# RoboEden/flatland-marl

Hardware: AMD Instinct MI355X
Metric: agent-steps/sec (batched envs) + tree-obs build ms/step (higher is better)
Workload: dtype int32; 1 GPU; cfg2: 256 envs x 30x30 / 20 agents / 3 cities (Round-2 Test_2); envs_per_gpu=256, agents=20, obs=cutils(31 nodes, pred 500) + upstream tree depth 2 (pred 30), actions=counter-hash uniform 0..4 generated on device, auto-reset at episode end, distinct_maps=8, dm_rebuild=at commit only, parallelism=envs sharded over 1 GPU(s), metrics all-reduce only, launch=one host call per kernel launch

## Files before the change

### flatland_marl_amd/csrc/fl_obs.hip

```cpp
#include <algorithm>
#include <stdio.h>
#include <stdlib.h>
#include <string.h>

#include "../../include/flatland_hip.h"
#include "fl_obs_layout.h"

int fl_obs_alloc(FlObsScratch &o, const FlDev &d, hipStream_t s, std::vector<void *> &allocs) {
    o.pred_cap = OBS_PRED_CAP;
    o.items_cap = (size_t)d.A * (o.pred_cap + 2 * OBS_FB_NB + 2);
    o.wl_cap = OBS_WL_HBM_ENTRIES;
    const size_t B = (size_t)d.B, BA = B * d.A;
    if (fl_alloc_zeroed(&o.path, BA * o.pred_cap, s, allocs) != hipSuccess ||
        fl_alloc_zeroed(&o.cell_items, B * o.items_cap, s, allocs, 64) != hipSuccess ||
        fl_alloc_zeroed(&o.dbg, B * 64, s, allocs) != hipSuccess || fl_alloc_zeroed(&o.bk_rel, B * (d.Rcap + 1) * OBS_BK_NB, s, allocs) != hipSuccess ||
        fl_alloc_zeroed(&o.wl, B * o.wl_cap, s, allocs) != hipSuccess || fl_alloc_zeroed(&o.label, (size_t)d.A, s, allocs) != hipSuccess ||
        fl_alloc_zeroed(&o.rowmask, BA, s, allocs) != hipSuccess || fl_alloc_zeroed(&o.cost, B, s, allocs) != hipSuccess ||
        fl_alloc_zeroed(&o.order, B, s, allocs) != hipSuccess) return FL_ERR_HIP;
    o.rows_out = nullptr; o.rows_depth = 0; o.keep_rows = 0;
    int dev = 0, n_cu = 0;
    if (hipGetDevice(&dev) != hipSuccess || hipDeviceGetAttribute(&n_cu, hipDeviceAttributeMultiprocessorCount, dev) != hipSuccess) return FL_ERR_HIP;
    o.n_cu = n_cu;
    o.order_age = 0;
    return FL_OK;
}

bool fl_obs_no_compact() { static const bool v = getenv("FL_OBS_NO_COMPACT") != nullptr; return v; }
static bool obs_no_fix() { static const bool v = getenv("FL_OBS_NO_FIX") != nullptr; return v; }
static bool obs_no_split() { static const bool v = getenv("FL_OBS_NO_SPLIT") != nullptr; return v; }
static bool obs_no_cutils_merge() { static const bool v = getenv("FL_OBS_NO_CUTILS_MERGE") != nullptr; return v; }
static bool obs_verbose_on() { static const bool v = getenv("FL_OBS_VERBOSE") != nullptr; return v; }
static bool obs_no_wl_head() { static const bool v = getenv("FL_OBS_NO_WL_HEAD") != nullptr; return v; }

__global__ __launch_bounds__(1024) void k_env_order(int B, const uint32_t *__restrict__ cost, int *__restrict__ order) {
    __shared__ unsigned int hist[1024];
    __shared__ unsigned int wsum[16];
    __shared__ unsigned int cmax;
    const int tid = threadIdx.x;
    hist[tid] = 0;
    if (tid == 0) cmax = 1;
    __syncthreads();
    unsigned int m = 0;
    for (int b = tid; b < B; b += 1024) m = max(m, cost[b]);
    for (int off = 32; off > 0; off >>= 1) m = max(m, (unsigned int)__shfl_down((int)m, off));
    if ((tid & 63) == 0) atomicMax(&cmax, m);
    __syncthreads();
// ... 375 lines not shown
    record[0] = -1;
    return d.A <= 1024 && pred_depth + 2 <= o.pred_cap && pred_depth <= 510;
}
static int obs_run(FlObsScratch &o, const FlDev &d, ObsArgs &P, const int *h_R, hipStream_t s, int record[FL_OBS_LAUNCH_WORDS]) {
    ObsOptions accepted = {};
    const int n_fit = obs_configure(d, P, accepted, h_R);
    if (n_fit < 0) return FL_ERR_ARG;
    o.last_fix = P.fix; o.last_split = P.split; o.last_fit = n_fit;
    uint4 *const rowmask = o.rowmask;
    struct Restore { FlObsScratch &o; uint4 *m; ~Restore() { o.rowmask = m; } } restore{o, rowmask};
    if (P.tw_t) {
        P.keep_rows = o.keep_rows && o.rows_out == P.tree_out && o.rows_depth == P.max_depth;
        o.rows_out = P.tree_out; o.rows_depth = P.max_depth;
        if (!o.keep_rows || P.max_depth > 3) { o.rowmask = nullptr; P.keep_rows = 0; o.rows_out = nullptr; }
    }
    obs_verbose(P);
    obs_keep_verify(d, P, rowmask, s);
    FlObsScratch u = o;
    if (P.merged == 1) u.order = nullptr;
    else u = fl_obs_env_order(o, d, s);
    const int rc = obs_launch(d, u, P, s);
    if (rc == FL_OK) obs_record_launch(P, accepted, record);
    return rc;
}

int fl_launch_obs_cutils(FlObsScratch &o, const FlDev &d, int max_nodes, int pred_depth, const FlObsCutilsOut &out, hipStream_t s,
                         int record[FL_OBS_LAUNCH_WORDS], const int16_t *label_dev, int out64) {
    if (!obs_begin(o, d, pred_depth, record) || max_nodes > FL_OBS_MAX_NODES) return FL_ERR_ARG;
    ObsArgs P = {};
    P.label = label_dev;
// ... 31 lines not shown

int fl_obs_config_of_fused(const FlDev &d, int pred_depth, int max_depth, int tree_pred, int out[11], int wide) {
    ObsArgs P = {};
    obs_cutils_args(P, 31, pred_depth, wide);
    if (max_depth > 0) obs_tree_args(d, P, max_depth, tree_pred, nullptr);
    else obs_alone_args(d, P);
    ObsOptions q = {};
    if (obs_configure(d, P, q, nullptr) < 0) return FL_ERR_ARG;
    if (obs_verbose_on()) {
        fprintf(stderr, "  options {nt %d, wl_bytes %d, tab %d, nh %d, tmask %d, dual %d, items %d, snext %d, partial %d, bk_room %d, own_filter %d, fb %d, raw %d, items_cap %d, wl_head %d}; "
                        "shape {merged %d, tw_c %d, tw_t %d, tpw_t %d, tree_pred %d}; bk %d tshift %d wl_occ_div %d\n",
                q.nt, q.wl_bytes, q.tab, q.nh, q.tmask, q.dual, q.items, q.snext, q.partial, q.bk_room, q.own_filter, q.fb, q.raw, q.items_cap, q.wl_head,
                P.merged, P.tw_c, P.tw_t, P.tpw_t, P.tree_pred, P.bk, P.tshift, P.wl_occ_div);
        static const char *names[L_COUNT] = {"cellw", "nbr", "snext", "rkey", "slot_agent", "slot_ready", "cell_target", "a_speed", "a_vpos", "a_pos", "a_tslot",
            "a_target", "a_malf", "a_tpc", "a_tq", "a_tq2", "a_raw", "rtype", "a_lp", "a_n", "a_srank", "a_dir", "a_state", "a_free", "a_dead", "misc", "team_meta", "node_tables",
            "csr", "items", "wl", "partial", "tmask", "tmask2", "nh", "csr2", "tmaskb", "tmaskb2", "items2", "a_lp2", "a_tpc2", "bkrel", "seg", "dm", "hop8"};
        for (int k = 0; k < L_COUNT; k++) {
            if (P.L.off[k] == L_ABSENT) continue;
            unsigned next = P.L.total;
            for (int j = 0; j < L_COUNT; j++) if (P.L.off[j] != L_ABSENT && P.L.off[j] > P.L.off[k] && P.L.off[j] < next) next = P.L.off[j];
            fprintf(stderr, "  %-12s %7u B\n", names[k], next - P.L.off[k]);
        }
    }
    out[0] = P.L.nt; out[1] = (int)P.L.total; out[2] = P.L.tab_lds; out[3] = P.L.off[L_NH] != L_ABSENT; out[4] = P.L.wl_bytes;
    out[5] = P.use_tmask + 2 * (P.L.off[L_TMASK2] != L_ABSENT);
    out[6] = P.dual_index; out[7] = P.L.off[L_ITEMS] != L_ABSENT ? P.L.items_cap : 0;
    out[8] = P.merged; out[9] = P.compact_t; out[10] = P.fix;
    return FL_OK;
}
```

### flatland_marl_amd/csrc/fl_obs_body.h

```cpp
#pragma once
#include "fl_obs_trees.h"

__device__ __forceinline__ int obs_env_of_workgroup(const FlObsScratch &S) { return __builtin_amdgcn_readfirstlane(S.order ? S.order[blockIdx.x] : (int)blockIdx.x); }

template <bool CUTILS, int VAR, int STAGE, int MERGED = 0, int FIX = 0, bool UP = true>
__device__ __forceinline__ void obs_body(const FlDev &d, const FlObsScratch &S, const ObsArgs &P_launch) {
    using FixT = ObsFixed<FIX != 0 ? FIX : 1>;
    ObsArgs P_local = P_launch;
    if (FIX != 0) {
        P_local.max_nodes = FixT::max_nodes; P_local.pred_depth = FixT::pred_depth; P_local.tree_pred = FixT::shape.tree_pred;
        P_local.tshift = obs_fixed_tshift<FIX != 0 ? FIX : 1>(d.A);
        if (FixT::max_depth != 0) {
            P_local.max_depth = FixT::max_depth;
            P_local.n_tree_nodes = FixT::max_depth == 2 ? 21 : 85;
        }
    }
    const ObsArgs &P = P_local;
    constexpr bool TAB_LDS = (VAR & 1) != 0, WL_HBM = (VAR & 2) != 0;
    const int b = MERGED == 1 ? (int)blockIdx.x : obs_env_of_workgroup(S), tid = threadIdx.x,
              nt = MERGED == 3 ? 512 : (FIX != 0 || MERGED == 1 || MERGED == 2) ? OBS_NT : (int)blockDim.x;
    const int A = (FIX != 0 && FixT::agents != 0) ? FixT::agents : d.A, R = d.R[b], NS = R * 4, K = d.K[b], U = d.U[b];
    const int Rcap = d.Rcap, Scap = Rcap * 4;
    const int lane = tid & 63, wave = tid >> 6;

// ... 31 lines not shown
    uint8_t *a_dead = LDS_AT(uint8_t, L_A_DEAD);
    int *misc = LDS_AT(int, L_MISC);
    int *team_meta = LDS_AT(int, L_TEAM_META);
    int *wave_scr = LDS_AT(int, L_WAVE_SCR);
    int *csr = LDS_AT(int, L_CSR);
    uint32_t *items_lds = LDS_OPT(uint32_t, L_ITEMS);
    uint32_t *wl_lds = WL_HBM ? nullptr : LDS_AT(uint32_t, L_WL);
    int *partial = (WL_HBM || L_OFF(L_PARTIAL) != L_ABSENT) ? LDS_AT(int, L_PARTIAL) : reinterpret_cast<int *>(wl_lds);
    const int wl_entries = WL_HBM ? OBS_WL_HBM_ENTRIES : L_FIELD(wl_bytes) / 8;
    unsigned long long *tmask = LDS_OPT(unsigned long long, L_TMASK);
    uint16_t *nh_lds = LDS_OPT(uint16_t, L_NH);
    int *csr2 = LDS_OPT(int, L_CSR2);
    unsigned long long *tmaskb = LDS_OPT(unsigned long long, L_TMASKB);
    unsigned long long *tmask_m2 = LDS_OPT(unsigned long long, L_TMASK2), *tmaskb_m2 = LDS_OPT(unsigned long long, L_TMASKB2);
    uint32_t *items2 = LDS_OPT(uint32_t, L_ITEMS2);
    uint16_t *a_lp2 = LDS_OPT(uint16_t, L_A_LP2);
    uint16_t *a_tpc2 = LDS_OPT(uint16_t, L_A_TPC2);
    double *a_tq2 = LDS_OPT(double, L_A_TQ2);
    uint32_t *a_raw = LDS_OPT(uint32_t, L_A_RAW);
    uint8_t *rtype_lds = LDS_OPT(uint8_t, L_RTYPE);
    uint4 *seg_lds = TAB_LDS ? LDS_AT(uint4, L_SEG) : nullptr;
    uint16_t *dm_lds = TAB_LDS ? LDS_AT(uint16_t, L_DM) : nullptr;
    uint16_t *hop8_lds = TAB_LDS ? LDS_AT(uint16_t, L_HOP8) : nullptr;
    const int tb = __builtin_amdgcn_readfirstlane(d.tab[b]);
    const uint4 *gseg = d.seg + (size_t)tb * Scap;
    const uint16_t *gdm = d.dm + (size_t)tb * d.Ucap * Scap;
    const uint16_t *ghop8 = d.hop8 + (size_t)tb * d.Ucap * Scap;
    const uint16_t *gnh = d.nh + (size_t)tb * d.Ucap * Rcap;

    const int T = d.T[b], tnow = d.t[b];
// ... 134 lines not shown
    X.wl_cf = X.wl_occ + X.wl_occ_cap; X.wl_cf_cap = wl_entries - X.wl_occ_cap;
    {
        const int head_entries = (WL_HBM && MERGED != 0 && L_OFF(L_WL) != L_ABSENT) ? L_FIELD(wl_head) / 8 : 0;
        uint2 *head = head_entries > 0 ? LDS_AT(uint2, L_WL) : nullptr;
        X.wl_head_occ = head; X.wl_head_occ_n = head_entries / p_wl_occ_div;
        X.wl_head_cf = head + X.wl_head_occ_n; X.wl_head_cf_n = head_entries - X.wl_head_occ_n;
    }
    X.wl_cnt = misc + 8;
    X.long_lists = misc + 11;
    X.tshift = X.Tn <= 64 ? 0 : P.tshift;
    constexpr bool merged = MERGED != 0;
    constexpr int ROUND = MERGED == 3 ? 16 : 32;
    X.n_cu = ROUND; X.round_base = 0;
    X.u_csr_end = csr2; X.u_items = items2; X.u_tmask = tmaskb; X.a_tq2 = a_tq2;
    X.tmask_m2 = merged ? tmask_m2 : nullptr; X.u_tmask_m2 = tmaskb_m2;
    X.path = S.path + (size_t)b * A * OBS_PRED_CAP; X.pred_cap = OBS_PRED_CAP;
    X.a_lp = a_lp; X.a_lp2 = a_lp2; X.a_tpc2 = a_tpc2;
    X.u_Tn = P.tree_pred + 1; X.u_tshift = X.u_Tn <= 64 ? 0 : P.tshift;

    OBS_STAMP(1);
    auto phase1a = [&]() __attribute__((always_inline)) {
        if (A <= 64) {
            const int i = lane;
            bool active = false, fr = false;
            unsigned long long blockers = 0;
            if (i < A && is_on_map(a_state[i]) && !a_dead[i]) {
                active = true;
                const uint32_t bits = nibble(cw_bits(X, a_pos[i]), a_dir[i]);
                if (bits == 0) fr = true;
                for (uint32_t m = 0; m < 4; m++) {
// ... 204 lines not shown
    }
    OBS_STAMP(2);
    if (X.Tn > 0) {
        const bool dual = UP && CUTILS && STAGE == 1 && p_dual_index && P.tree_pred >= 0;
        const bool reuse = STAGE == 2 && p_dual_index && misc[4] != 0;
        const int Tn2 = P.tree_pred + 1, tshift2 = Tn2 <= 64 ? 0 : P.tshift;
        const bool bk = CUTILS && STAGE != 2 && p_bk != 0 && X.Tn > 64 && X.tmask != nullptr;
        const bool bk_lds = bk && p_bk == 2;
        const int bk_nb = p_bk_nb, bk_shift = p_bk_shift;
        const int bk_w = bk_lds ? bk_nb + 2 : bk_nb;
        uint32_t *bkc = bk_lds ? LDS_AT(uint32_t, L_BKREL) : reinterpret_cast<uint32_t *>(wave_scr);
        if (!reuse) {
            for (int k = tid; k <= K; k += nt) csr[k] = 0;
            if (tid == 0) misc[11] = 0;
            if (X.tmask) for (int k = tid; k <= K; k += nt) { tmask[k] = 0ull; if (X.tmask_m2) tmask_m2[k] = 0ull; }
            if (bk) for (int k = tid; k < (bk_lds ? K * bk_w / 2 : ((K + 1) * bk_nb + 1) / 2); k += nt) bkc[k] = 0u;
        }
        if (dual) for (int k = tid; k <= K; k += nt) { csr2[k] = 0; if (p_use_tmask) tmaskb[k] = 0ull; if (X.tmask_m2) tmaskb_m2[k] = 0ull; }
        if (STAGE != 2 && tid < 64) { team_meta[64 + tid] = 1; team_meta[192 + tid] = 1; }
        __syncthreads();
        const int pred_depth = my_pred_depth;
        if (STAGE != 2) {
        const int w_first = (nt >> 6) - nw_walk, wsel = wave - w_first;
        if (do_p1 && p1_beside_walk && wave == w_first - 1) {
            phase1a();
#ifdef FL_OBS_TIMING
            if (lane == 0) atomicMax((unsigned long long *)&X.dbg[20], (unsigned long long)wall_clock64());
#endif
        }
        if (wsel >= 0) __builtin_amdgcn_s_setprio(3);
        const int n_max = CUTILS ? pred_depth + 1 : max(pred_depth, 1);
        for (int base = 0; wsel >= 0 && base < A; base += 8 * nw_walk) {
            const int slot = lane >> 3, j = lane & 7;
// ... 399 lines not shown
                } else {
                    tlo = k * tpc;
                    span = tpc;
                }
                const bool to_end = k == lp || tlo + span - 1 >= tlast;
                const int key = key_of(X, (int)(w >> 2));
                if (X.tmask) {
                    const int b1 = tb_of(tlo, X.tshift), b2 = tb_of(to_end ? tlast : tlo + span - 1, X.tshift);
                    const unsigned long long bits = ((2ull << b2) - 1ull) & ~((1ull << b1) - 1ull);
                    if (X.tmask_m2) {
                        const unsigned long long seen = atomicOr(&tmask[key], bits);
                        if (seen & bits) atomicOr(&tmask_m2[key], seen & bits);
                    } else {
                        atomicOr(&tmask[key], bits);
                    }
                }
                const uint32_t item = IT_MAKE(lab ? (int)lab[i] : i, tlo, to_end, span, dprev, dnext, w & 3u);
                if (bk) {
                    const int thi = to_end ? tlast : tlo + span - 1;
                    int b1 = min(tlo >> bk_shift, bk_nb - 1), b2 = min(thi >> bk_shift, bk_nb - 1);
                    if (bk_lds && to_end) b1 = b2 = bk_nb;
                    for (int bb = b1; bb <= b2; bb++) {
                        const int kb = key * bk_w + bb;
                        const uint32_t old = atomicAdd(&bkc[kb >> 1], (kb & 1) ? 0x10000u : 1u);
                        csr_items[csr[key] + (int)((kb & 1) ? (old >> 16) : (old & 0xFFFFu))] = item;
                    }
                } else {
                    const int slot = atomicAdd(&csr[key], 1);
                    csr_items[slot] = item;
                }
                if (k <= lp2) {
                    const int tlo2 = k * tpc2, tlast2 = Tn2 - 1;
                    const bool to_end2 = k == lp2 || tlo2 + tpc2 - 1 >= tlast2;
                    const uint32_t dnext2 = k < lp2 ? dnext : (w & 3u);
                    if (p_use_tmask) {
                        const int b1 = tb_of(tlo2, tshift2), b2 = tb_of(to_end2 ? tlast2 : tlo2 + tpc2 - 1, tshift2);
                        const unsigned long long bits = ((2ull << b2) - 1ull) & ~((1ull << b1) - 1ull);
                        if (X.tmask_m2) {
                            const unsigned long long seen = atomicOr(&tmaskb[key], bits);
                            if (seen & bits) atomicOr(&tmaskb_m2[key], seen & bits);
                        } else {
                            atomicOr(&tmaskb[key], bits);
                        }
                    }
                    const int slot2 = atomicAdd(&csr2[key], 1);
                    items2[slot2] = IT_MAKE(i, tlo2, to_end2, tpc2, dprev, dnext2, w & 3u);
                }
            }
            }
        }
        __syncthreads();
#ifdef FL_OBS_TIMING
        if (STAGE != 2 && tid == 0) {
            P.dbg[(size_t)b * 64 + 57] = (long long)wall_clock64();
            int wp = 0;
            for (int i = 0; i < A; i++) wp += a_n[i];
            P.dbg[(size_t)b * 64 + 58] = misc[2];
// ... 86 lines not shown
```

### flatland_marl_amd/csrc/fl_obs_ctx.h

```cpp
#pragma once
#include <stdio.h>
#include <type_traits>

#include "../../include/flatland_hip.h"
#include "fl_obs_layout.h"

struct ObsCtx {
    int A, R;
    int SS;
    const uint32_t *cellw;
    const uint16_t *nbr;
    const uint16_t *snext;
    const uint16_t *rkey;
    const int *slot_agent;
    const int *slot_ready;
    const uint32_t *cell_target;
    const uint16_t *a_vpos;
    const uint8_t *a_dir, *a_state;
    const uint16_t *a_malf;
    const double *a_speed;
    const uint16_t *a_tpc;
    const double *a_tq;
    const uint16_t *a_tslot;
    const uint16_t *a_target;
// ... 13 lines not shown
    int wl_occ_cap, wl_cf_cap;
    uint2 *wl_head_occ, *wl_head_cf;
    int wl_head_occ_n, wl_head_cf_n;
    int *wl_cnt;
    const int *long_lists;
    const unsigned long long *tmask;
    int tshift;
    int n_cu;
    int round_base;
    const int *u_csr_end;
    const uint32_t *u_items;
    const unsigned long long *u_tmask;
    int u_Tn, u_tshift;
    const double *a_tq2;
    const unsigned long long *tmask_m2, *u_tmask_m2;
    const uint16_t *path;
    int pred_cap;
    const uint16_t *a_lp, *a_lp2, *a_tpc2;
    long long *dbg;
    int dbg_base;
};

#ifndef OBS_NT_LEVEL
#define OBS_NT_LEVEL 2
#endif
typedef float obs_f4_t __attribute__((ext_vector_type(4)));
typedef double obs_d2_t __attribute__((ext_vector_type(2)));
__device__ __forceinline__ void fill_store_d2(double *p, double a, double b) {
#if OBS_NT_LEVEL >= 1
    const obs_d2_t v = {a, b};
// ... 22 lines not shown
template <typename T>
__device__ __forceinline__ void out_store(T *p, T v) {
#if OBS_NT_LEVEL >= 3
    __builtin_nontemporal_store(v, p);
#else
    *p = v;
#endif
}

__device__ __forceinline__ int tb_of(int t, int ts) { return min(t >> ts, 63); }

__device__ __forceinline__ uint32_t cw_bits(const ObsCtx &X, int r) { return X.cellw[r] & 0xFFFFu; }
__device__ __forceinline__ uint32_t cw_slot(const ObsCtx &X, int r) { return X.cellw[r] >> 16; }
__device__ __forceinline__ uint32_t cw_load(const ObsCtx &X, int r) { return X.cellw[r]; }
__device__ __forceinline__ int key_of(const ObsCtx &X, int r) { return X.rkey ? (int)X.rkey[r] : r; }
template <int PB>
__device__ __forceinline__ bool pb_cu(const ObsCtx &X, int team) { return PB == 3 ? true : PB == 2 ? team < X.n_cu : PB == 1; }
template <int PB>
__device__ __forceinline__ int pb_handle(const ObsCtx &X, const int *team_meta, int team) {
    return PB == 3 ? X.round_base + team : PB == 2 ? X.round_base + (team < X.n_cu ? team : team - X.n_cu) : team_meta[128 + team];
}
template <int PB>
__device__ __forceinline__ int pt_of(const ObsCtx &X, bool cu, int handle, int tot) {
    if (PB == 2 && !cu) return (int)((double)tot * X.a_tq2[handle]);
    return cu ? (int)((float)tot * (float)X.a_tq[handle]) : (int)((double)tot * X.a_tq[handle]);
}
struct ListRange { int lo, n1, lo2, n; };
template <bool TWO>
__device__ __forceinline__ int list_index(const ListRange &R, int v) { return (TWO && v >= R.n1) ? R.lo2 + (v - R.n1) : R.lo + v; }
template <int PB>
// ... 114 lines not shown
```

### flatland_marl_amd/csrc/fl_obs_layout.h

```cpp
#pragma once
#include <stdint.h>

#include "fl_obs.h"

#define OBS_NT 1024
#ifndef CF_CHUNK_LDS
#define CF_CHUNK_LDS 16
#endif
#ifndef CF_CHUNK_HBM
#define CF_CHUNK_HBM 8
#endif
#ifndef CF_FIRST_HBM
#define CF_FIRST_HBM 8
#endif
#ifndef OBS_GLB_BATCH
#define OBS_GLB_BATCH 8
#endif
#ifndef OBS_WL_OCC_DIV
#define OBS_WL_OCC_DIV 6
#endif
#ifndef OBS_TSHIFT
#define OBS_TSHIFT 1
#endif
#ifndef CF_DIRECT
// ... 27 lines not shown
#define N_NONE 0xFFFFu
enum { ND_TARGET = 1, ND_SWITCH = 2, ND_DEAD_END = 4, ND_TERMINAL = 8, ND_ZERO = 16, ND_PHANTOM = 32  };

#define OBS_CAP_C 32
#define OBS_CAP_T_COMPACT 16

__host__ __device__ constexpr int obs_scr_words(int nwaves, int A, int tw_c, int tw_t, int tpw_t) {
    const int tpw_c = tw_c > N_WORDS_C * OBS_CAP_C ? 1 : 2;
    const int n_c = tpw_c * nwaves <= A ? tpw_c * nwaves : A + 1, n_t = tpw_t * nwaves <= A ? tpw_t * nwaves : A + 1;
    const int w_c = n_c * tw_c, w_t = n_t * tw_t;
    return w_c > w_t ? w_c : w_t;
}

enum { L_CELLW = 0, L_NBR, L_SNEXT, L_RKEY, L_SLOT_AGENT, L_SLOT_READY, L_CELL_TARGET, L_A_SPEED, L_A_VPOS, L_A_POS, L_A_TSLOT,
       L_A_TARGET, L_A_MALF, L_A_TPC, L_A_TQ, L_A_TQ2, L_A_RAW, L_RTYPE, L_A_LP, L_A_N, L_A_SRANK, L_A_DIR, L_A_STATE, L_A_FREE, L_A_DEAD, L_MISC, L_TEAM_META, L_WAVE_SCR,
       L_CSR, L_ITEMS, L_WL, L_PARTIAL, L_TMASK, L_TMASK2, L_NH, L_CSR2, L_TMASKB, L_TMASKB2, L_ITEMS2, L_A_LP2, L_A_TPC2, L_BKREL, L_SEG, L_DM, L_HOP8, L_COUNT };
#define L_ABSENT 0xFFFFFFFFu
struct ObsLayout {
    unsigned off[L_COUNT];
    unsigned total;
    int nt;
    int wl_bytes;
    int wl_head;
    int tab_lds;
    int items_cap, items2_cap;
};

struct ObsOptions { int nt, wl_bytes, tab, nh, tmask, dual, items, snext, partial, bk_room, own_filter, fb, raw, items_cap, wl_head; };
struct ObsDims { int Rcap, A, Ucap, rkey; };
struct ObsShape { int merged, tw_c, tw_t, tpw_t, tree_pred; };

__host__ __device__ constexpr unsigned obs_al16(unsigned long long bytes) { return (unsigned)((bytes + 15ull) & ~15ull); }
__host__ __device__ constexpr ObsLayout obs_layout_c(const ObsDims &d, const ObsShape &P, const ObsOptions &o) {
    ObsLayout L = {};
    for (int k = 0; k < L_COUNT; k++) L.off[k] = L_ABSENT;
    unsigned off = 0;
#define OBS_PUT(which, bytes) do { L.off[which] = off; off += obs_al16((unsigned long long)(bytes)); } while (0)
    const unsigned long long R = (unsigned long long)d.Rcap, NS = R * 4, A = (unsigned long long)d.A, K1 = R + 1, U = (unsigned long long)d.Ucap;
    OBS_PUT(L_CELLW, R * 4);
    OBS_PUT(L_NBR, NS * 2);
    if (o.snext) OBS_PUT(L_SNEXT, NS * 2);
    if (d.rkey) OBS_PUT(L_RKEY, R * 2);
    OBS_PUT(L_SLOT_AGENT, A * 4); OBS_PUT(L_SLOT_READY, A * 4);
    OBS_PUT(L_CELL_TARGET, ((R + 31) / 32) * 4);
    OBS_PUT(L_A_SPEED, A * 8); OBS_PUT(L_A_TQ, A * 8);
    if (P.merged && o.raw) { OBS_PUT(L_A_RAW, A * 32); OBS_PUT(L_RTYPE, R); }
// ... 16 lines not shown
    L.items2_cap = (int)(i2 < OBS_ITEMS2_CAP ? i2 : OBS_ITEMS2_CAP);
    if (o.items) OBS_PUT(L_ITEMS, (unsigned long long)L.items_cap * 4);
    if (o.wl_bytes) OBS_PUT(L_WL, o.wl_bytes);
    else if (o.wl_head) OBS_PUT(L_WL, o.wl_head);
    if (o.partial || !o.wl_bytes) OBS_PUT(L_PARTIAL, (unsigned long long)o.nt * 4);
    if (o.tmask) OBS_PUT(L_TMASK, K1 * 8);
    if (o.tmask && P.merged && o.own_filter) OBS_PUT(L_TMASK2, K1 * 8);
    if (o.dual) {
        OBS_PUT(L_CSR2, K1 * 4);
        if (o.tmask) OBS_PUT(L_TMASKB, K1 * 8);
        if (o.tmask && P.merged && o.own_filter) OBS_PUT(L_TMASKB2, K1 * 8);
        OBS_PUT(L_ITEMS2, (unsigned long long)(L.items2_cap > 4 ? L.items2_cap : 4) * 4);
        OBS_PUT(L_A_LP2, A * 2); OBS_PUT(L_A_TPC2, A * 2); OBS_PUT(L_A_TQ2, A * 8);
    }
    if (o.fb) OBS_PUT(L_BKREL, K1 * (OBS_FB_NB + 2) * 2);
    if (o.nh || o.tab) OBS_PUT(L_NH, U * R * 2);
    if (o.tab) { OBS_PUT(L_SEG, NS * 16); OBS_PUT(L_DM, U * NS * 2); OBS_PUT(L_HOP8, U * NS * 2); }
#undef OBS_PUT
    L.total = off;
    L.nt = o.nt; L.wl_bytes = o.wl_bytes; L.tab_lds = o.tab; L.wl_head = o.wl_bytes ? 0 : o.wl_head;
    return L;
}

#define OBS_FIX3_RCAP 680
#define OBS_FIX4_RCAP 2816
#define OBS_FIX4_A 432
#define OBS_FIX3_WL_HEAD (10 * 1024)
#ifndef OBS_WL_HEAD_MAX
#define OBS_WL_HEAD_MAX (32 * 1024)
#endif
// ... 166 lines not shown
    int32_t *adjacency, *node_order, *edge_order;
    uint8_t *valid;
    double *props;
    double *tree_out;
    int n_tree_nodes;
    long long *dbg;
    int tw_c, tw_t, tpw_t;
    int compact_t;
    int use_tmask;
    int tshift;
    int dual_index;
    int bk;
    int bk_nb, bk_shift;
    int merged;
    int wl_occ_div;
    int fix;
    const int16_t *label;
    int keep_mode;
    int keep_rows;
    int out64;
    int cutils_alone;
    int wide;
    int fix_allowed;
    const int *h_R;
    int split;
    ObsLayout L;
};

template <int MODE>
int fl_obs_launch_mode(int var, const FlDev &d, const FlObsScratch &o, const ObsArgs &P, hipStream_t s);
// ... 3 lines not shown
```

### flatland_marl_amd/csrc/fl_obs_passb.h

```cpp
#pragma once
#include "fl_obs_ctx.h"

__device__ __forceinline__ void occ_event(const ObsCtx &X, bool CUTILS, int *sc, int cap, int node, uint32_t sl, uint32_t d, int tot) {
    const int ag = X.slot_agent[sl];
    if (ag < 0) return;
    atomicMin(&nt_w(sc, cap, N_OA, node), tot);
    const int mf = (int)X.a_malf[ag];
    if (mf > 0) {
        if (CUTILS) atomicOr(&nt_w(sc, cap, N_RM, node), 1 << 16);
        else atomicMax(&nt_w(sc, cap, N_MALF, node), mf);
    }
    const int rd = X.slot_ready[sl];
    const int radd = rd > 0 ? (CUTILS ? rd - 1 : rd) : 0;
    if (radd) atomicAdd(&nt_w(sc, cap, N_RM, node), radd);
    if (X.a_dir[ag] == d) {
        atomicAdd(&nt_w(sc, cap, N_CNT, node), 1);
        const double sp = CUTILS ? (double)(float)X.a_speed[ag] : X.a_speed[ag];
        if (sp < 1.0) atomicMin(reinterpret_cast<unsigned int *>(&nt_w(sc, cap, N_MS, node)), ((unsigned int)X.a_srank[ag] << 10) | (unsigned int)ag);
    } else {
        atomicAdd(&nt_w(sc, cap, N_CNT, node), 1 << 16);
    }
}

template <int PB, bool ITL, bool TWO>
// ... 169 lines not shown
    for (int c = NCH - 1; c >= 0; c--)
        if (real[c]) first_real = c * TEAM + __ffsll((long long)real[c]) - 1;
    return run_base;
}

template <int PB, int CAP>
__device__ __forceinline__ int *team_table(const ObsCtx &X, int *scr0, int team_words, int team) {
    if (PB == 3) return scr0 + team * (N_WORDS_C * 32);
    if (PB == 2) {
        const int u = team - X.n_cu;
        return u < 0 ? scr0 + team * (N_WORDS_C * 32) : scr0 + X.n_cu * (N_WORDS_C * 32) + (u >> 1) * (N_WORDS_T * 32) + (u & 1) * 16;
    }
    return scr0 + team * team_words;
}

struct NoLateWork { __device__ __forceinline__ void operator()() const {} };

template <int PB, int CAP, bool ITL, typename LATE = NoLateWork, bool TWO = false>
__device__ __forceinline__ void wg_pass_b(const ObsCtx &X, int tid, int nt, int n_teams, int *scr0, int team_words,
                                          const int *team_meta, const LATE &late = LATE()) {
    if (tid == 0) { X.wl_cnt[0] = 0; X.wl_cnt[1] = 0; X.wl_cnt[2] = 0; }
    __syncthreads();
    const int lane = tid & 63;
    const int tv = lane < n_teams ? team_meta[lane] : 0;
    int tincl = tv;
#pragma unroll
    for (int off = 1; off < 64; off <<= 1) { const int u = __shfl_up(tincl, off); if (lane >= off) tincl += u; }
    const int total = __builtin_amdgcn_readlane(tincl, 63);
    const int q = (total + nt - 1) / nt;
    int pos = tid * q;
// ... 32 lines not shown
            const int i1 = nt_r(vs, cap, N_INCL, m1) & 0xFFFFFF, i2 = nt_r(vs, cap, N_INCL, m2) & 0xFFFFFF, i3 = nt_r(vs, cap, N_INCL, m3) & 0xFFFFFF;
            if (i1 > lpos) hi = m1;
            else if (i2 > lpos) { lo = m1 + 1; hi = m2; }
            else if (i3 > lpos) { lo = m2 + 1; hi = m3; }
            else lo = min(m3 + 1, hi);
        }
        int node = lo;
        int target;
        double tq;
        bool cu;
        const unsigned long long *tmask_t = X.tmask, *tmask2_t = X.tmask_m2;
        int Tn_t = X.Tn, tshift_t = X.tshift;
        const bool self_filter = PB >= 2 && X.tmask_m2 != nullptr;
        const uint16_t *path_t = X.path;
        int lp_t = 0, tpc_t = 1;
        auto enter_team = [&]() __attribute__((always_inline)) {
            target = X.a_target[handle];
            cu = pb_cu<PB>(X, team);
            tq = (PB == 2 && !cu) ? X.a_tq2[handle] : X.a_tq[handle];
            if (PB == 2) { tmask_t = cu ? X.tmask : X.u_tmask; Tn_t = cu ? X.Tn : X.u_Tn; tshift_t = cu ? X.tshift : X.u_tshift; }
            if (PB >= 2 && self_filter) {
                tmask2_t = cu ? X.tmask_m2 : X.u_tmask_m2;
                path_t = X.path + (size_t)handle * X.pred_cap;
                lp_t = cu ? X.a_lp[handle] : X.a_lp2[handle];
                tpc_t = cu ? X.a_tpc[handle] : X.a_tpc2[handle];
            }
        };
        enter_team();
        int left, cell, tot, nxt;
        uint32_t dd;
        {
            const uint32_t inw = (uint32_t)nt_r(vs, cap, N_INCL, node), tvw = (uint32_t)nt_r(vs, cap, N_TV, node);
            const int nvis = nt_vis(tvw), incl = (int)(inw & 0xFFFFFFu);
            const int k = lpos - (incl - nvis);
            const uint32_t st = skip_cells(X, (uint32_t)nt_r(vs, cap, N_SE, node) & 0xFFFFu, k);
            cell = (int)(st >> 2); dd = st & 3u;
#ifdef FL_OBS_TIMING
            dbg_skip = k;
#endif
            tot = nt_tot(tvw) + k;
            left = nvis - k;
            nxt = (int)(inw >> 24);
        }
#ifdef FL_OBS_TIMING
        if (X.dbg && lane == 0) atomicMax((unsigned long long *)&X.dbg[24], (unsigned long long)((long long)wall_clock64() - dbg_t1));
#endif
        auto walk = [&](auto fast_tag) __attribute__((always_inline)) {
        constexpr bool FAST = decltype(fast_tag)::value;
        const bool has_snext = FAST || X.snext != nullptr, has_tmask = FAST || X.tmask != nullptr;
        uint32_t cw = 0, sn = 0, ct = 0, n_inw = 0, own_w = 0, n_se = 0, n_tv = 0;
        unsigned long long tm = 0, tm2 = 0;
        int c_hi = 0, c_lo = 0;
        auto request = [&]() __attribute__((always_inline)) {
            if (FAST && self_filter) own_w = path_t[min(tot, lp_t)];
            cw = cw_load(X, cell);
            if (has_snext) sn = X.snext[((uint32_t)cell << 2) | dd];
            if (FAST || X.Tn > 0) {
                const int key = FAST ? cell : key_of(X, cell);
                if (has_tmask) { tm = tmask_t[key]; if (FAST && self_filter) tm2 = tmask2_t[key]; }
                else { c_hi = X.csr_end[key]; c_lo = key > 0 ? X.csr_end[key - 1] : 0; }
            }
            if (PB != 1 && PB != 3) ct = X.cell_target[cell >> 5];
            if (left == 1 && nxt < nn) {
                n_se = (uint32_t)nt_r(vs, cap, N_SE, nxt); n_tv = (uint32_t)nt_r(vs, cap, N_TV, nxt);
                n_inw = (uint32_t)nt_r(vs, cap, N_INCL, nxt);
            }
        };
        request();
        while (true) {
            const int e_cell = cell, e_tot = tot, e_node = node, e_handle = handle;
            const uint32_t e_dd = dd;
            const bool e_cu = cu;
            int *sc = const_cast<int *>(vs);
            constexpr int e_cap = cap;
// ... 4 lines not shown
            int pt = 0;
            if ((FAST || X.Tn > 0) && tot < Tn_t) {
                pt = cu ? (int)((float)tot * (float)tq) : (int)((double)tot * tq);
                if (pt < Tn_t) {
                    if (has_tmask) {
                        const int b1 = tb_of(max(pt - 1, 0), tshift_t), b2 = tb_of(min(pt + 1, Tn_t - 1), tshift_t);
                        unsigned long long others = tm;
                        if (FAST && self_filter && tot >= 1 && tot <= lp_t && (int)(own_w >> 2) == cell) {
                            const int tlast = Tn_t - 1;
                            const int tlo = cu ? (tot - 1) * tpc_t + 1 : tot * tpc_t, te = tlo + tpc_t - 1;
                            const int thi = (tot == lp_t || te >= tlast) ? tlast : te;
                            const int o1 = tb_of(tlo, tshift_t), o2 = tb_of(thi, tshift_t);
                            others = (tm & ~(((2ull << o2) - 1ull) & ~((1ull << o1) - 1ull))) | tm2;
                        }
                        cand = ((uint32_t)(others >> b1) & ((2u << (b2 - b1)) - 1u)) != 0u;
                    } else {
                        cand = c_hi > c_lo;
                    }
                }
            }
            const bool tgt_hit = !cu && ((ct >> (cell & 31)) & 1u) && cell != target;
            const bool to_cf = cand && has_tmask;
            const unsigned long long m_occ = __ballot(occ), m_cf = __ballot(to_cf);
            const unsigned long long resv = wl_reserve2_issue(X.wl_cnt, m_occ, m_cf);
            pos++;
            left--;
            const bool more = pos < end;
            if (more) {
                if (left > 0) {
                    const uint32_t s2 = has_snext ? sn : chain_next(X, ((uint32_t)cell << 2) | dd, cw & 0xFFFFu);
// ... 57 lines not shown
#endif
    for (int e = tid; e < n_occ; e += nt) {
        const uint2 w = wl_occ_get(X, e);
        const int cell = (int)((w.x & 0xFFFFFFu) >> 2), team = (int)(w.x >> 24);
        constexpr int cap = PB >= 2 ? 32 : CAP;
        int *sc = team_table<PB, CAP>(X, scr0, team_words, team);
        occ_event(X, pb_cu<PB>(X, team), sc, cap, (int)(w.y >> 24), cw_slot(X, cell), w.x & 3u, (int)(w.y & 0xFFFFFFu));
    }
    WAVE_MARK(X, 12, -1);
    WL_ACC(X, 0);
    if (*X.long_lists == 0) {
        for (int e = tid; e < n_cf; e += nt) {
            const uint2 w = wl_cf_get(X, e);
            const int cell = (int)((w.x & 0xFFFFFFu) >> 2), team = (int)(w.x >> 24);
            const int handle = pb_handle<PB>(X, team_meta, team), tot = (int)(w.y & 511u);
            const bool cu = pb_cu<PB>(X, team);
            const int pt = pt_of<PB>(X, cu, handle, tot);
            const ListRange R = list_range<PB>(X, cu, cell, pt);
#ifdef FL_OBS_COUNTS
            const uint32_t f = R.n > 0 ? conflict_flags<PB, ITL, TWO>(X, cu, handle, cell, w.x & 3u, pt, R, 0, R.n) : 0u;
            if (X.dbg) {
                atomicAdd((unsigned long long *)&X.dbg[X.dbg_base + 27], (unsigned long long)R.n);
                if (tb_of(pt, X.tshift) >= 63) atomicAdd((unsigned long long *)&X.dbg[X.dbg_base + 28], 1ull);
                if (f & 7u) atomicAdd((unsigned long long *)&X.dbg[X.dbg_base + 29], 1ull);
                if (conflict_hit(f)) atomicAdd((unsigned long long *)&X.dbg[X.dbg_base + 30], 1ull);
                if (!(f & 7u) && (f & 64u)) atomicAdd((unsigned long long *)&X.dbg[X.dbg_base + 31], 1ull);
            }
            if (conflict_hit(f)) {
#else
            if (R.n > 0 && conflict_hit(conflict_flags<PB, ITL, TWO>(X, cu, handle, cell, w.x & 3u, pt, R, 0, R.n))) {
// ... 17 lines not shown
        const int e = e0 + tid;
        int nch = 0, cell = 0, handle = 0, tot = 0, pt = 0, team = 0, np = 0;
        ListRange R = {0, 0, 0, 0};
        bool cu = PB == 1;
        uint2 w = make_uint2(0u, 0u);
        uint32_t fl = 0;
        if (e < n_cf) {
            w = wl_cf_get(X, e);
            cell = (int)((w.x & 0xFFFFFFu) >> 2);
            team = (int)(w.x >> 24);
            handle = pb_handle<PB>(X, team_meta, team);
            tot = (int)(w.y & 511u);
            cu = pb_cu<PB>(X, team);
            pt = pt_of<PB>(X, cu, handle, tot);
            R = list_range<PB>(X, cu, cell, pt);
            nch = 1 + min(max(R.n - CF_FIRST + CF_CHUNK - 1, 0) / CF_CHUNK, 62);
            const uint32_t f = R.n > 0 ? conflict_flags<PB, ITL, TWO>(X, cu, handle, cell, w.x & 3u, pt, R, 0, min(R.n, CF_FIRST)) : 0u;
#ifdef FL_OBS_COUNTS
            if (X.dbg) {
                atomicAdd((unsigned long long *)&X.dbg[X.dbg_base + 27], (unsigned long long)R.n);
                if (tb_of(pt, X.tshift) >= 63) atomicAdd((unsigned long long *)&X.dbg[X.dbg_base + 28], 1ull);
                if (f & 7u) atomicAdd((unsigned long long *)&X.dbg[X.dbg_base + 29], 1ull);
                if (conflict_hit(f)) atomicAdd((unsigned long long *)&X.dbg[X.dbg_base + 30], 1ull);
                if (!(f & 7u) && (f & 64u)) atomicAdd((unsigned long long *)&X.dbg[X.dbg_base + 31], 1ull);
            }
#endif
            fl = f & 63u;
        }
        for (int j = 1; __any(j < nch); j++) {
            const bool want = j < nch;
// ... 17 lines not shown
    WL_ACC(X, 1);
    late();
    WL_ACC(X, 2);
    __syncthreads();
    WAVE_MARK(X, 14, -1);
    WL_ACC(X, 3);
    const int n_cf2 = min(X.wl_cnt[1], X.wl_cf_cap);
    for (int e = n_cf + tid; e < n_cf2; e += nt) {
        const uint2 w = wl_cf_get(X, e);
        const int cell = (int)((w.x & 0xFFFFFFu) >> 2), team = (int)(w.x >> 24);
        const int first = (int)((w.y >> 6) & 0x1FFFFu), chunk = (int)(w.y & 63u), tot = (int)(w.y >> 23);
        const int handle = pb_handle<PB>(X, team_meta, team);
        const bool cu = pb_cu<PB>(X, team);
        const int pt = pt_of<PB>(X, cu, handle, tot);
        const ListRange R = list_range<PB>(X, cu, cell, pt);
        const uint32_t f = conflict_flags<PB, ITL, TWO>(X, cu, handle, cell, w.x & 3u, pt, R, CF_FIRST + (chunk - 1) * CF_CHUNK, chunk == 62 ? R.n : min(R.n, CF_FIRST + chunk * CF_CHUNK));
        const uint32_t old = wl_cf_done(X, first, (f & 63u) << 15);
        if (((old >> 9) & 63u) == 1u && conflict_hit((old >> 15) & 63u)) {
            constexpr int cap = PB >= 2 ? 32 : CAP;
            int *sc = team_table<PB, CAP>(X, scr0, team_words, team);
            atomicMin(&nt_w(sc, cap, N_PC, (int)(old >> 24)), (int)(old & 511u));
        }
    }
    WL_ACC(X, 4);
    WL_ACC(X, 5);
    __syncthreads();
}
```

Before: 115.1 million agent-steps/s.

## Add per-direction conflict masks and skip conflict checks on already-settled nodes

Builds per-cell, per-direction conflict bitmasks (cmask and cmaskb) in LDS while agent paths are inserted. The tree walk uses them to drop candidate conflicts whose direction cannot actually conflict, so fewer cells are pushed to the conflict worklist. Conflict-list scans are also skipped when the team's node already holds a conflict at or before the current time. The cost is extra LDS space, extra atomics during path insertion, and more complex filtering logic whose correctness depends on the direction rules.

```diff
diff --git a/flatland_marl_amd/csrc/fl_obs.hip b/flatland_marl_amd/csrc/fl_obs.hip
--- a/flatland_marl_amd/csrc/fl_obs.hip
+++ b/flatland_marl_amd/csrc/fl_obs.hip
@@ -30,6 +30,7 @@
 static bool obs_no_split() { static const bool v = getenv("FL_OBS_NO_SPLIT") != nullptr; return v; }
 static bool obs_no_cutils_merge() { static const bool v = getenv("FL_OBS_NO_CUTILS_MERGE") != nullptr; return v; }
 static bool obs_verbose_on() { static const bool v = getenv("FL_OBS_VERBOSE") != nullptr; return v; }
+static bool obs_no_cf_dirs() { static const bool v = getenv("FL_OBS_NO_CF_DIRS") != nullptr; return v; }
 static bool obs_no_wl_head() { static const bool v = getenv("FL_OBS_NO_WL_HEAD") != nullptr; return v; }
 
 __global__ __launch_bounds__(1024) void k_env_order(int B, const uint32_t *__restrict__ cost, int *__restrict__ order) {
@@ -435,6 +436,7 @@
         o.rows_out = P.tree_out; o.rows_depth = P.max_depth;
         if (!o.keep_rows || P.max_depth > 3) { o.rowmask = nullptr; P.keep_rows = 0; o.rows_out = nullptr; }
     }
+    P.no_cf_dirs = obs_no_cf_dirs();
     obs_verbose(P);
     obs_keep_verify(d, P, rowmask, s);
     FlObsScratch u = o;
@@ -496,7 +498,7 @@
                 P.merged, P.tw_c, P.tw_t, P.tpw_t, P.tree_pred, P.bk, P.tshift, P.wl_occ_div);
         static const char *names[L_COUNT] = {"cellw", "nbr", "snext", "rkey", "slot_agent", "slot_ready", "cell_target", "a_speed", "a_vpos", "a_pos", "a_tslot",
             "a_target", "a_malf", "a_tpc", "a_tq", "a_tq2", "a_raw", "rtype", "a_lp", "a_n", "a_srank", "a_dir", "a_state", "a_free", "a_dead", "misc", "team_meta", "node_tables",
-            "csr", "items", "wl", "partial", "tmask", "tmask2", "nh", "csr2", "tmaskb", "tmaskb2", "items2", "a_lp2", "a_tpc2", "bkrel", "seg", "dm", "hop8"};
+            "csr", "items", "wl", "partial", "tmask", "tmask2", "nh", "csr2", "tmaskb", "tmaskb2", "items2", "a_lp2", "a_tpc2", "bkrel", "seg", "dm", "hop8", "cmask", "cmaskb"};
         for (int k = 0; k < L_COUNT; k++) {
             if (P.L.off[k] == L_ABSENT) continue;
             unsigned next = P.L.total;
diff --git a/flatland_marl_amd/csrc/fl_obs_body.h b/flatland_marl_amd/csrc/fl_obs_body.h
--- a/flatland_marl_amd/csrc/fl_obs_body.h
+++ b/flatland_marl_amd/csrc/fl_obs_body.h
@@ -69,6 +69,13 @@
     unsigned long long *tmaskb = LDS_OPT(unsigned long long, L_TMASKB);
     unsigned long long *tmask_m2 = LDS_OPT(unsigned long long, L_TMASK2), *tmaskb_m2 = LDS_OPT(unsigned long long, L_TMASKB2);
     uint32_t *items2 = LDS_OPT(uint32_t, L_ITEMS2);
+#ifdef FL_OBS_COUNTS
+    const bool cf_off = false;
+#else
+    const bool cf_off = P.no_cf_dirs != 0;
+#endif
+    unsigned long long *cmask = cf_off ? nullptr : LDS_OPT(unsigned long long, L_CMASK);
+    uint32_t *cmaskb = (cf_off || P.tree_pred + 1 > 32) ? nullptr : LDS_OPT(uint32_t, L_CMASKB);
     uint16_t *a_lp2 = LDS_OPT(uint16_t, L_A_LP2);
     uint16_t *a_tpc2 = LDS_OPT(uint16_t, L_A_TPC2);
     double *a_tq2 = LDS_OPT(double, L_A_TQ2);
@@ -233,6 +240,10 @@
     X.n_cu = ROUND; X.round_base = 0;
     X.u_csr_end = csr2; X.u_items = items2; X.u_tmask = tmaskb; X.a_tq2 = a_tq2;
     X.tmask_m2 = merged ? tmask_m2 : nullptr; X.u_tmask_m2 = tmaskb_m2;
+    X.cmask = cmask; X.u_cmask = cmaskb;
+#ifdef FL_OBS_COUNTS
+    X.cf_count_only = P.no_cf_dirs != 0;
+#endif
     X.path = S.path + (size_t)b * A * OBS_PRED_CAP; X.pred_cap = OBS_PRED_CAP;
     X.a_lp = a_lp; X.a_lp2 = a_lp2; X.a_tpc2 = a_tpc2;
     X.u_Tn = P.tree_pred + 1; X.u_tshift = X.u_Tn <= 64 ? 0 : P.tshift;
@@ -467,9 +478,11 @@
             for (int k = tid; k <= K; k += nt) csr[k] = 0;
             if (tid == 0) misc[11] = 0;
             if (X.tmask) for (int k = tid; k <= K; k += nt) { tmask[k] = 0ull; if (X.tmask_m2) tmask_m2[k] = 0ull; }
+            if (cmask) for (int k = tid; k < NS; k += nt) cmask[k] = 0ull;
             if (bk) for (int k = tid; k < (bk_lds ? K * bk_w / 2 : ((K + 1) * bk_nb + 1) / 2); k += nt) bkc[k] = 0u;
         }
         if (dual) for (int k = tid; k <= K; k += nt) { csr2[k] = 0; if (p_use_tmask) tmaskb[k] = 0ull; if (X.tmask_m2) tmaskb_m2[k] = 0ull; }
+        if (dual && cmaskb) for (int k = tid; k < NS; k += nt) cmaskb[k] = 0u;
         if (STAGE != 2 && tid < 64) { team_meta[64 + tid] = 1; team_meta[192 + tid] = 1; }
         __syncthreads();
         const int pred_depth = my_pred_depth;
@@ -899,6 +912,12 @@
                     } else {
                         atomicOr(&tmask[key], bits);
                     }
+                    if (cmask) {
+                        const uint32_t dirs = cf_dirs_of(cw_bits(X, (int)(w >> 2)), cf_against(w & 3u) | cf_against(dnext) | cf_against(dprev), a_state[i] == ST_DONE);
+#pragma unroll
+                        for (uint32_t dw = 0; dw < 4; dw++)
+                            if ((dirs >> dw) & 1u) atomicOr(&cmask[((uint32_t)key << 2) | dw], bits);
+                    }
                 }
                 const uint32_t item = IT_MAKE(lab ? (int)lab[i] : i, tlo, to_end, span, dprev, dnext, w & 3u);
                 if (bk) {
@@ -926,6 +945,12 @@
                             if (seen & bits) atomicOr(&tmaskb_m2[key], seen & bits);
                         } else {
                             atomicOr(&tmaskb[key], bits);
+                        }
+                        if (cmaskb) {
+                            const uint32_t dirs = cf_dirs_of(cw_bits(X, (int)(w >> 2)), cf_against(w & 3u), a_state[i] == ST_DONE);
+#pragma unroll
+                            for (uint32_t dw = 0; dw < 4; dw++)
+                                if ((dirs >> dw) & 1u) atomicOr(&cmaskb[((uint32_t)key << 2) | dw], (uint32_t)bits);
                         }
                     }
                     const int slot2 = atomicAdd(&csr2[key], 1);
diff --git a/flatland_marl_amd/csrc/fl_obs_ctx.h b/flatland_marl_amd/csrc/fl_obs_ctx.h
--- a/flatland_marl_amd/csrc/fl_obs_ctx.h
+++ b/flatland_marl_amd/csrc/fl_obs_ctx.h
@@ -51,6 +51,11 @@
     int u_Tn, u_tshift;
     const double *a_tq2;
     const unsigned long long *tmask_m2, *u_tmask_m2;
+    const unsigned long long *cmask;
+    const uint32_t *u_cmask;
+#ifdef FL_OBS_COUNTS
+    bool cf_count_only;
+#endif
     const uint16_t *path;
     int pred_cap;
     const uint16_t *a_lp, *a_lp2, *a_tpc2;
@@ -103,6 +108,16 @@
 __device__ __forceinline__ uint32_t cw_slot(const ObsCtx &X, int r) { return X.cellw[r] >> 16; }
 __device__ __forceinline__ uint32_t cw_load(const ObsCtx &X, int r) { return X.cellw[r]; }
 __device__ __forceinline__ int key_of(const ObsCtx &X, int r) { return X.rkey ? (int)X.rkey[r] : r; }
+__device__ __forceinline__ uint32_t cf_against(uint32_t cd) { return 1u << (3u - ((cd + 2u) & 3u)); }
+__device__ __forceinline__ uint32_t cf_dirs_of(uint32_t bits16, uint32_t against, bool done) {
+    uint32_t dirs = 0;
+#pragma unroll
+    for (uint32_t d = 0; d < 4; d++) {
+        const uint32_t nib = nibble(bits16, d);
+        if (nib != 0 && (done || (nib & against & ~cf_against(d)) != 0)) dirs |= 1u << d;
+    }
+    return dirs;
+}
 template <int PB>
 __device__ __forceinline__ bool pb_cu(const ObsCtx &X, int team) { return PB == 3 ? true : PB == 2 ? team < X.n_cu : PB == 1; }
 template <int PB>
diff --git a/flatland_marl_amd/csrc/fl_obs_layout.h b/flatland_marl_amd/csrc/fl_obs_layout.h
--- a/flatland_marl_amd/csrc/fl_obs_layout.h
+++ b/flatland_marl_amd/csrc/fl_obs_layout.h
@@ -65,7 +65,7 @@
 
 enum { L_CELLW = 0, L_NBR, L_SNEXT, L_RKEY, L_SLOT_AGENT, L_SLOT_READY, L_CELL_TARGET, L_A_SPEED, L_A_VPOS, L_A_POS, L_A_TSLOT,
        L_A_TARGET, L_A_MALF, L_A_TPC, L_A_TQ, L_A_TQ2, L_A_RAW, L_RTYPE, L_A_LP, L_A_N, L_A_SRANK, L_A_DIR, L_A_STATE, L_A_FREE, L_A_DEAD, L_MISC, L_TEAM_META, L_WAVE_SCR,
-       L_CSR, L_ITEMS, L_WL, L_PARTIAL, L_TMASK, L_TMASK2, L_NH, L_CSR2, L_TMASKB, L_TMASKB2, L_ITEMS2, L_A_LP2, L_A_TPC2, L_BKREL, L_SEG, L_DM, L_HOP8, L_COUNT };
+       L_CSR, L_ITEMS, L_WL, L_PARTIAL, L_TMASK, L_TMASK2, L_NH, L_CSR2, L_TMASKB, L_TMASKB2, L_ITEMS2, L_A_LP2, L_A_TPC2, L_BKREL, L_SEG, L_DM, L_HOP8, L_CMASK, L_CMASKB, L_COUNT };
 #define L_ABSENT 0xFFFFFFFFu
 struct ObsLayout {
     unsigned off[L_COUNT];
@@ -81,6 +81,7 @@
 struct ObsDims { int Rcap, A, Ucap, rkey; };
 struct ObsShape { int merged, tw_c, tw_t, tpw_t, tree_pred; };
 
+__host__ __device__ constexpr bool obs_has_cf_dirs(const ObsShape &P, const ObsOptions &o) { return P.merged == 1 && o.tmask != 0; }
 __host__ __device__ constexpr unsigned obs_al16(unsigned long long bytes) { return (unsigned)((bytes + 15ull) & ~15ull); }
 __host__ __device__ constexpr ObsLayout obs_layout_c(const ObsDims &d, const ObsShape &P, const ObsOptions &o) {
     ObsLayout L = {};
@@ -127,6 +128,7 @@
         OBS_PUT(L_A_LP2, A * 2); OBS_PUT(L_A_TPC2, A * 2); OBS_PUT(L_A_TQ2, A * 8);
     }
     if (o.fb) OBS_PUT(L_BKREL, K1 * (OBS_FB_NB + 2) * 2);
+    if (obs_has_cf_dirs(P, o)) { OBS_PUT(L_CMASK, NS * 8); if (o.dual) OBS_PUT(L_CMASKB, NS * 4); }
     if (o.nh || o.tab) OBS_PUT(L_NH, U * R * 2);
     if (o.tab) { OBS_PUT(L_SEG, NS * 16); OBS_PUT(L_DM, U * NS * 2); OBS_PUT(L_HOP8, U * NS * 2); }
 #undef OBS_PUT
@@ -323,6 +325,7 @@
     int bk_nb, bk_shift;
     int merged;
     int wl_occ_div;
+    int no_cf_dirs;
     int fix;
     const int16_t *label;
     int keep_mode;
diff --git a/flatland_marl_amd/csrc/fl_obs_passb.h b/flatland_marl_amd/csrc/fl_obs_passb.h
--- a/flatland_marl_amd/csrc/fl_obs_passb.h
+++ b/flatland_marl_amd/csrc/fl_obs_passb.h
@@ -207,6 +207,16 @@
     return scr0 + team * team_words;
 }
 
+template <int PB, int CAP>
+__device__ __forceinline__ bool cf_settled(const ObsCtx &X, int *scr0, int team_words, int team, int node, int tot) {
+#ifdef OBS_NO_PC_SKIP
+    return false;
+#else
+    constexpr int cap = PB >= 2 ? 32 : CAP;
+    return nt_r(team_table<PB, CAP>(X, scr0, team_words, team), cap, N_PC, node) <= tot;
+#endif
+}
+
 struct NoLateWork { __device__ __forceinline__ void operator()() const {} };
 
 template <int PB, int CAP, bool ITL, typename LATE = NoLateWork, bool TWO = false>
@@ -269,6 +279,8 @@
         const bool self_filter = PB >= 2 && X.tmask_m2 != nullptr;
         const uint16_t *path_t = X.path;
         int lp_t = 0, tpc_t = 1;
+        const bool cf_any = PB >= 2 && (X.cmask != nullptr || X.u_cmask != nullptr);
+        bool cf_t = false;
         auto enter_team = [&]() __attribute__((always_inline)) {
             target = X.a_target[handle];
             cu = pb_cu<PB>(X, team);
@@ -280,6 +292,7 @@
                 lp_t = cu ? X.a_lp[handle] : X.a_lp2[handle];
                 tpc_t = cu ? X.a_tpc[handle] : X.a_tpc2[handle];
             }
+            if (PB >= 2 && cf_any) cf_t = cu ? X.cmask != nullptr : X.u_cmask != nullptr;
         };
         enter_team();
         int left, cell, tot, nxt;
@@ -304,7 +317,7 @@
         constexpr bool FAST = decltype(fast_tag)::value;
         const bool has_snext = FAST || X.snext != nullptr, has_tmask = FAST || X.tmask != nullptr;
         uint32_t cw = 0, sn = 0, ct = 0, n_inw = 0, own_w = 0, n_se = 0, n_tv = 0;
-        unsigned long long tm = 0, tm2 = 0;
+        unsigned long long tm = 0, tm2 = 0, cm = 0;
         int c_hi = 0, c_lo = 0;
         auto request = [&]() __attribute__((always_inline)) {
             if (FAST && self_filter) own_w = path_t[min(tot, lp_t)];
@@ -313,6 +326,9 @@
             if (FAST || X.Tn > 0) {
                 const int key = FAST ? cell : key_of(X, cell);
                 if (has_tmask) { tm = tmask_t[key]; if (FAST && self_filter) tm2 = tmask2_t[key]; }
+                if (FAST && cf_any && cf_t) {
+                    if (cu) cm = X.cmask[((uint32_t)cell << 2) | dd]; else cm = (unsigned long long)X.u_cmask[((uint32_t)cell << 2) | dd];
+                }
                 else { c_hi = X.csr_end[key]; c_lo = key > 0 ? X.csr_end[key - 1] : 0; }
             }
             if (PB != 1 && PB != 3) ct = X.cell_target[cell >> 5];
@@ -347,6 +363,14 @@
                             others = (tm & ~(((2ull << o2) - 1ull) & ~((1ull << o1) - 1ull))) | tm2;
                         }
                         cand = ((uint32_t)(others >> b1) & ((2u << (b2 - b1)) - 1u)) != 0u;
+                        if (FAST && cf_any && cf_t) {
+                            const bool can = ((uint32_t)(cm >> b1) & ((2u << (b2 - b1)) - 1u)) != 0u;
+#ifdef FL_OBS_COUNTS
+                            if (cand && !can && X.dbg) atomicAdd((unsigned long long *)&X.dbg[46], 1ull);
+                            if (!X.cf_count_only)
+#endif
+                            cand = cand && can;
+                        }
                     } else {
                         cand = c_hi > c_lo;
                     }
@@ -434,6 +458,7 @@
             const uint2 w = wl_cf_get(X, e);
             const int cell = (int)((w.x & 0xFFFFFFu) >> 2), team = (int)(w.x >> 24);
             const int handle = pb_handle<PB>(X, team_meta, team), tot = (int)(w.y & 511u);
+            if (cf_settled<PB, CAP>(X, scr0, team_words, team, (int)(w.y >> 24), tot)) continue;
             const bool cu = pb_cu<PB>(X, team);
             const int pt = pt_of<PB>(X, cu, handle, tot);
             const ListRange R = list_range<PB>(X, cu, cell, pt);
@@ -481,6 +506,7 @@
             cu = pb_cu<PB>(X, team);
             pt = pt_of<PB>(X, cu, handle, tot);
             R = list_range<PB>(X, cu, cell, pt);
+            if (cf_settled<PB, CAP>(X, scr0, team_words, team, (int)(w.y >> 24), tot)) R.n = 0;
             nch = 1 + min(max(R.n - CF_FIRST + CF_CHUNK - 1, 0) / CF_CHUNK, 62);
             const uint32_t f = R.n > 0 ? conflict_flags<PB, ITL, TWO>(X, cu, handle, cell, w.x & 3u, pt, R, 0, min(R.n, CF_FIRST)) : 0u;
 #ifdef FL_OBS_COUNTS
@@ -528,7 +554,8 @@
         const bool cu = pb_cu<PB>(X, team);
         const int pt = pt_of<PB>(X, cu, handle, tot);
         const ListRange R = list_range<PB>(X, cu, cell, pt);
-        const uint32_t f = conflict_flags<PB, ITL, TWO>(X, cu, handle, cell, w.x & 3u, pt, R, CF_FIRST + (chunk - 1) * CF_CHUNK, chunk == 62 ? R.n : min(R.n, CF_FIRST + chunk * CF_CHUNK));
+        const bool settled = cf_settled<PB, CAP>(X, scr0, team_words, team, (int)(wl_cf_get(X, first).y >> 24), tot);
+        const uint32_t f = settled ? 0u : conflict_flags<PB, ITL, TWO>(X, cu, handle, cell, w.x & 3u, pt, R, CF_FIRST + (chunk - 1) * CF_CHUNK, chunk == 62 ? R.n : min(R.n, CF_FIRST + chunk * CF_CHUNK));
         const uint32_t old = wl_cf_done(X, first, (f & 63u) << 15);
         if (((old >> 9) & 63u) == 1u && conflict_hit((old >> 15) & 63u)) {
             constexpr int cap = PB >= 2 ? 32 : CAP;
```

Measured after the change: 121.7 million agent-steps/s, median of 6. +5.8%, better.
